# ygjwd12345/UCD

Hardware: AMD Instinct MI355X
Metric: images/sec (whole node) per UCD train step, VOC 15-5 step-1, 513^2 bs=24 (higher is better)
Workload: dtype bf16

## Files before the change

include/ucd_hip.h:

```cpp
#ifndef UCD_HIP_H
#define UCD_HIP_H

#include <stddef.h>
#include <stdint.h>

#ifdef __cplusplus
extern "C" {
#endif

#define UCD_VERSION 100

typedef void* ucd_stream_t;
typedef void* ucd_comm_t;

enum ucd_dtype { UCD_F32 = 0, UCD_BF16 = 1 };
enum ucd_act { UCD_ACT_IDENTITY = 0, UCD_ACT_LEAKY_RELU = 1, UCD_ACT_ELU = 2  };
#define UCD_ACT_MASK 0xff
#define UCD_NORM_ABS_GAMMA 0x100
enum ucd_pixcon_precision { UCD_PIXCON_F32 = 0, UCD_PIXCON_F16 = 1, UCD_PIXCON_F16_SPLIT = 2 };
enum ucd_error {
  UCD_OK = 0,
  UCD_EINVAL = -1,
  UCD_EALIGN = -2,
  UCD_EWORKSPACE = -3,
// ... 276 lines not shown

int ucd_conv3_tap_plan(int B, int H, int W, int dilation, int tile_rows, int* perm, int* masks, int* n_classes);
int ucd_conv3_tap_classes(int mode);
int ucd_conv3_tap_plans_resident(void);
int ucd_conv3_tap_stats(long long* launches, int* last_tile_rows, int* last_class_ordered);

int ucd_conv1x1_stats_finalize(const float* partial, int M, int C, const float* weight, float* running_mean,
                               float* running_var, float momentum, float eps, float* buf, float* pack, int flags,
                               ucd_stream_t stream);

int ucd_abn_reduce_partials(const float* partial, int tiles, int C, float* sums, float* sums_copy, const float* weight,
                            int flags, ucd_stream_t stream);

size_t ucd_conv1x1_wgrad_workspace_bytes(int M, int N, int K);
int ucd_conv1x1_wgrad(const void* dy, int ld_dy, const void* a, int lda, int M, int N, int K,
                      const float* in_mean, const float* in_scale, const float* in_shift, int in_act, float in_slope,
                      void* dw, void* workspace, size_t workspace_bytes, ucd_stream_t stream);

int ucd_abn_sync_finalize(const float* gathered, int world, int M, int C, const float* weight, float* running_mean,
                          float* running_var, float momentum, float eps, float* buf, int flags, ucd_stream_t stream);

int ucd_stem_conv7x7(const float* x, long long sb, long long sc, long long sh, long long sw, int B, int H, int W, const void* w,
                     void* z, ucd_stream_t stream);

int ucd_stem_conv_pool(const float* x, long long sb, long long sc, long long sh, long long sw, int B, int H, int W, const void* w,
                       const float* mean, const float* scale, const float* beta, int act, float slope, void* out, ucd_stream_t stream);
int ucd_stem_pooled_size(int n);
size_t ucd_stem_pool_workspace_bytes(int C);
int ucd_stem_apply_pool(const void* z, int B, int H, int W, int C, const float* mean, const float* scale, const float* beta, int act,
                        float slope, void* out, uint8_t* idx, ucd_stream_t stream);
int ucd_stem_pool_backward(const void* z, const void* dpool, const uint8_t* idx, int B, int H, int W, int C, const float* mean,
                           const float* invstd, const float* scale, const float* beta, const float* weight, float* sums, float count,
                           int act, float slope, void* dz, void* workspace, size_t workspace_bytes, int phase, ucd_stream_t stream);

size_t ucd_conv_wgrad_workspace_bytes(int M, int N, int K, int taps);
int ucd_conv_wgrad(const void* dz, int ld_dz, const void* x, int ld_x, int M, int N, int K, int taps, int H, int W, int dilation,
                   void* dw, float* dw32, int accumulate32, void* workspace, size_t workspace_bytes, ucd_stream_t stream);
int ucd_conv_wgrad_strided(const void* dz, int ld_dz, const void* x, int ld_x, int M, int N, int K, int taps, int H, int W,
                           int dilation, int stride, void* dw, float* dw32, int accumulate32, void* workspace, size_t workspace_bytes,
                           ucd_stream_t stream);
int ucd_conv_wgrad_ex(const void* dz, int ld_dz, const void* x, int ld_x, int M, int N, int K, int taps, int H, int W, int dilation,
                      int stride, void* dw, float* dw32, int accumulate32, void* workspace, size_t workspace_bytes, int flags,
                      ucd_stream_t stream);
int ucd_conv_wgrad_defer(int mode);
int ucd_conv_wgrad_mode(void);
int ucd_conv_wgrad_flush(ucd_stream_t stream);
int ucd_conv_wgrad_drop(ucd_stream_t stream);
int ucd_conv_wgrad_drop_all(void);

int ucd_flip_weights_batched(const void* src_flat, void* dst_flat, const int* blocks, int n_blocks, const long long* entries,
                             ucd_stream_t stream);
int ucd_flip_weights_batched64(const void* src_flat, void* dst_flat, const int* blocks, int n_blocks, const long long* entries,
                               ucd_stream_t stream);

int ucd_transpose_bf16(const void* src, int rows, int cols, void* dst, ucd_stream_t stream);

int ucd_conv_f32(const float* a, int lda, const float* w, int ldw, float* y, int ldy, int M, int N, int K, int taps, int H, int W,
                 int dilation, int accumulate, ucd_stream_t stream);
size_t ucd_conv_f32_wgrad_workspace_bytes(int M, int N, int K, int taps);
int ucd_conv_f32_wgrad(const float* dz, int ld_dz, const float* x, int ld_x, int M, int N, int K, int taps, int H, int W,
                       int dilation, float* dw, void* workspace, size_t workspace_bytes, ucd_stream_t stream);

#define UCD_SGD_MAX_GROUPS 8
typedef struct ucd_sgd_tensor {
  float* p;  const float* g;  float* m;  void* w16;
  long long n;
// ... 38 lines not shown
```

ucd_amd/abn.py:

```python
from __future__ import annotations

import os

from . import switches as _switches

import torch
import torch.distributed as dist
import torch.nn as nn
from torch.optim.optimizer import register_optimizer_step_post_hook

from . import hip
from .comm import direct_comm


def _act_code(name):
    try:
        return hip.ACT_CODES[name]
    except KeyError:
        raise RuntimeError(f"activation {name!r} is not supported by the HIP ABN (leaky_relu, elu, identity)") from None


_param_epoch = [0]


# ... 243 lines not shown
            sl = slice(o, o + c)
            dx = hip.empty_like_rows(x)
            hip.abn_bwd_apply(x, ld, dy[:, sl], ld_dy, None, 0, dx, c, None, 0, M, c, None, HW, mean[sl], invstd[sl],
                              scale[sl], shift[sl], weight[sl] if weight is not None else None,
                              sums[2 * o:2 * (o + c)], count, 0 if training else 1, act, slope)
            dxs.append(dx)
        return (dweight, dbias) + (None,) * 8 + tuple(dxs)


class _PlaneMean(torch.autograd.Function):

    @staticmethod
    def forward(ctx, x):
        x, M, Cc, HW, ld = hip.rows_view(x)
        B = x.shape[0]
        out = torch.empty(B, Cc, dtype=torch.float32, device=x.device)
        hip.plane_sum(x, ld, B, HW, Cc, 1.0 / HW, out)
        ctx.shape, ctx.dtype = x.shape, x.dtype
        return out.to(x.dtype).view(B, Cc, 1, 1)

    @staticmethod
    def backward(ctx, g):
        B, Cc, H, W = ctx.shape
        return (g.to(ctx.dtype) / (H * W)).expand(B, Cc, H, W)


def global_avg_pool(x):
    return _PlaneMean.apply(x)


class _StemABNPoolFunction(torch.autograd.Function):

    @staticmethod
    def forward(ctx, z, weight, bias, running_mean, running_var, training, momentum, eps, act, slope, group, eval_consts):
        B, Cc, H, W = z.shape
        M, HW = B * H * W, H * W
        zr, _, _, _, ld = hip.rows_view(z)
        dev = z.device
        world = _group_size(group) if training else 1
        sync = training and group is not False and (world > 1 or (_FORCE_SYNC and dist.is_initialized()))
        if training:
            buf = torch.empty(((8 + 2 * world) if sync else 6) * Cc, dtype=torch.float32, device=dev)
            if sync:
                pack = buf[6 * Cc:8 * Cc]
                hip.abn_sync_stats(zr, ld, M, Cc, None, HW, buf[:2 * Cc], buf[2 * Cc:3 * Cc], pack)
                comm = direct_comm(group)
                if comm is not None:
                    gathered = buf[8 * Cc:]
                    hip._check(hip.load().ucd_comm_all_gather(comm.handle, hip.ptr(pack), hip.ptr(gathered), 2 * Cc, hip.stream()),
                               "ucd_comm_all_gather")
                else:
                    gathered = _all_gather_stats(pack, world, group)
                hip.abn_sync_finalize(gathered, world, M, Cc, weight, running_mean, running_var, momentum, eps, buf, act)
            else:
                hip.abn_stats_finalize(zr, ld, M, Cc, None, HW, buf[:2 * Cc], buf[2 * Cc:3 * Cc], weight, running_mean, running_var,
                                       momentum, eps, buf[3 * Cc:4 * Cc], buf[4 * Cc:5 * Cc], buf[5 * Cc:6 * Cc], act)
            mean, invstd, scale = buf[3 * Cc:4 * Cc], buf[4 * Cc:5 * Cc], buf[5 * Cc:6 * Cc]
        else:
            mean, invstd, scale = running_mean, eval_consts[0], eval_consts[1]
        need_bwd = any(ctx.needs_input_grad[:3])
        out, idx = hip.stem_apply_pool(z, mean, scale, bias, act, slope, need_bwd)
        if need_bwd:
            ctx.save_for_backward(z, idx, weight, bias, mean, invstd, scale)
            ctx.cfg = (training, act, slope, group, world, sync, float(M * world))
        return out

    @staticmethod
    def backward(ctx, dp):
        z, idx, weight, bias, mean, invstd, scale = ctx.saved_tensors
        training, act, slope, group, world, sync, count = ctx.cfg
        if not training:
            raise RuntimeError("ucd_amd.abn: the fused stem has no frozen-statistics backward (fix_bn keeps the separate layers)")
        Cc = z.shape[1]
        if dp.dtype != z.dtype:
            dp = dp.to(z.dtype)
        if not dp.is_contiguous(memory_format=torch.channels_last):
            dp = dp.contiguous(memory_format=torch.channels_last)
        sums = torch.empty(2 * Cc, dtype=torch.float32, device=z.device)
        dz = torch.empty_like(z) if ctx.needs_input_grad[0] else None
        if not sync:
            hip.stem_pool_backward(z, dp, idx, mean, invstd, scale, bias, weight, sums, count, act, slope, dz, 3 if dz is not None else 1)
            dbias, dweight = sums[:Cc], sums[Cc:]
        else:
            hip.stem_pool_backward(z, dp, idx, mean, invstd, scale, bias, weight, sums, count, act, slope, None, 1)
            local = sums.clone()
            dbias, dweight = local[:Cc], local[Cc:]
            comm = direct_comm(group)
            if comm is not None:
                hip._check(hip.load().ucd_comm_all_reduce_sum(comm.handle, hip.ptr(sums), 2 * Cc, hip.stream()), "ucd_comm_all_reduce_sum")
            else:
                _all_reduce_sums(sums, group)
            if dz is not None:
                hip.stem_pool_backward(z, dp, idx, mean, invstd, scale, bias, weight, sums, count, act, slope, dz, 2)
        return (dz, dweight if weight is not None else None, dbias if bias is not None else None) + (None,) * 9


def stem_norm_pool(bn, z):
    import os
    if _switches.get("UCD_STEM_FOLD", "1") == "0" or not getattr(bn, "ucd_fused_abn", False):
        return None
    Cc = z.shape[1] if z.dim() == 4 else 0
    if not (z.is_cuda and z.dim() == 4 and z.dtype == torch.bfloat16 and z.is_contiguous(memory_format=torch.channels_last)
            and z.shape[2] > 2 and z.shape[3] > 2 and Cc % 8 == 0 and 2048 % max(Cc, 1) == 0
            and bn.activation in ("leaky_relu", "identity")):
        return None
    needs_grad = torch.is_grad_enabled() and (z.requires_grad or (bn.weight is not None and bn.weight.requires_grad))
    if needs_grad and not bn.training:
        return None
    act = _act_code(bn.activation) | (hip.NORM_ABS_GAMMA if bn._abs_gamma else 0)
    if bn.training:
        bn.__dict__.pop("_eval_cache", None)
    return _StemABNPoolFunction.apply(z, bn.weight, bn.bias, bn.running_mean, bn.running_var, bn.training, bn.momentum, bn.eps, act,
                                      bn.activation_param, bn._group(), None if bn.training else bn._eval_constants())


class ABN(nn.Module):

    ucd_fused_abn = True
    _inplace_contract = False
    _sync = False
    _abs_gamma = False

    def __init__(self, num_features, eps=1e-5, momentum=0.1, affine=True, activation="leaky_relu",
                 activation_param=0.01, group=None):
        super().__init__()
        self.num_features, self.eps, self.momentum, self.affine = num_features, eps, momentum, affine
        self.activation, self.activation_param = activation, activation_param
        self.group = group
        if affine:
            self.weight = nn.Parameter(torch.ones(num_features))
            self.bias = nn.Parameter(torch.zeros(num_features))
        else:
            self.register_parameter("weight", None)
            self.register_parameter("bias", None)
        self.register_buffer("running_mean", torch.zeros(num_features))
        self.register_buffer("running_var", torch.ones(num_features))

    def reset_parameters(self):
        nn.init.constant_(self.running_mean, 0)
        nn.init.constant_(self.running_var, 1)
        if self.affine:
            nn.init.constant_(self.weight, 1)
            nn.init.constant_(self.bias, 0)

    def _group(self):
        return self.group if self._sync else False
# ... 82 lines not shown
```

ucd_amd/backbone.py:

```python
from __future__ import annotations

import sys
from collections import OrderedDict
from functools import partial

import torch
import torch.nn as nn

from . import switches as _switches
from .blocks import Conv2d, ResidualBlock, try_index

_STAGE_DILATION = {16: (1, 1, 1, 2), 8: (1, 1, 2, 4)}


class GlobalAvgPool2d(nn.Module):

    def forward(self, inputs):
        return inputs.flatten(2).mean(dim=2)


class ResNet(nn.Module):
    def __init__(self, structure, bottleneck, norm_act=nn.BatchNorm2d, classes=0,
                 output_stride=16, keep_outputs=False):
        super().__init__()
# ... 19 lines not shown
                blocks[f"block{b + 1}"] = ResidualBlock(cin, width, norm_act=norm_act, stride=stride, dilation=d)
                cin = width[-1]
            self.add_module(f"mod{stage + 2}", nn.Sequential(blocks))
            width = tuple(2 * c for c in width)
        self.out_channels = cin

        if classes != 0:
            self.classifier = nn.Sequential(OrderedDict(
                [("avg_pool", GlobalAvgPool2d()), ("fc", nn.Linear(cin, classes))]))

    def _stem(self, x):
        m = self.mod1
        if hasattr(m, "pool1") and getattr(m.bn1, "ucd_fused_abn", False) and x.is_cuda:
            pool = m.pool1
            if (pool.kernel_size, pool.stride, pool.padding, pool.dilation, pool.ceil_mode) == (3, 2, 1, 1, False):
                from .abn import stem_norm_pool
                y = _stem_eval_fused(m.conv1, m.bn1, x)
                if y is not None:
                    return y
                z = _stem_conv(m.conv1, x)
                y = stem_norm_pool(m.bn1, z)
                return y if y is not None else pool(m.bn1(z))
        return m(x)

    def forward(self, x):
        outs = [self._stem(x)]
        for name in ("mod2", "mod3", "mod4", "mod5"):
            outs.append(getattr(self, name)(outs[-1]))
        if hasattr(self, "classifier"):
            outs.append(self.classifier(outs[-1]))
        return outs if self.keep_outputs else outs[-1]


class _StemConvFunction(torch.autograd.Function):

    @staticmethod
    def forward(ctx, x, w):
        from . import hip
        ctx.save_for_backward(x, w)
        return hip.stem_conv7x7(x, w)

    @staticmethod
    def backward(ctx, dz):
        x, w = ctx.saved_tensors
        dw = None
        if ctx.needs_input_grad[1]:
            xb = x.to(torch.bfloat16).contiguous(memory_format=torch.channels_last)
            dw = torch.ops.aten.convolution_backward(dz.contiguous(memory_format=torch.channels_last), xb, w, None, [2, 2], [3, 3],
                                                     [1, 1], False, [0, 0], 1, [False, True, False])[1]
        return None, dw


def _stem_conv(conv, x):
    w = conv.working_weight() if hasattr(conv, "working_weight") else None
    if w is None and x.is_cuda and torch.is_autocast_enabled() and torch.get_autocast_dtype("cuda") == torch.bfloat16:
        w = conv.weight.to(torch.bfloat16)
    if (w is None or not x.is_cuda or x.dim() != 4 or x.dtype != torch.float32 or x.requires_grad or conv.bias is not None
            or tuple(conv.weight.shape) != (64, 3, 7, 7) or conv.stride != (2, 2) or conv.padding != (3, 3)
            or conv.dilation != (1, 1) or w.dtype != torch.bfloat16 or not w.is_contiguous(memory_format=torch.channels_last)
            or _switches.get("UCD_OWN_STEM", "1") == "0"):
        return conv(x)
    if torch.is_grad_enabled() and w.requires_grad:
        return _StemConvFunction.apply(x, w)
    from . import hip
    return hip.stem_conv7x7(x, w)


def _stem_eval_fused(conv, bn, x):
    from . import abn as _abn
    if (torch.is_grad_enabled() or bn.training or _switches.get("UCD_STEM_EVAL_FUSED", "1") == "0" or _switches.get("UCD_OWN_STEM", "1") == "0"
            or _switches.get("UCD_STEM_FOLD", "1") == "0" or not getattr(bn, "ucd_fused_abn", False)
            or bn.activation not in ("leaky_relu", "identity")):
        return None
    w = conv.working_weight() if hasattr(conv, "working_weight") else None
    if w is None and x.is_cuda and torch.is_autocast_enabled() and torch.get_autocast_dtype("cuda") == torch.bfloat16:
        w = conv.weight.to(torch.bfloat16)
    if (w is None or not x.is_cuda or x.dim() != 4 or x.dtype != torch.float32 or conv.bias is not None
            or tuple(conv.weight.shape) != (64, 3, 7, 7) or conv.stride != (2, 2) or conv.padding != (3, 3) or conv.dilation != (1, 1)
            or w.dtype != torch.bfloat16 or not w.is_contiguous(memory_format=torch.channels_last) or x.shape[2] < 8 or x.shape[3] < 8):
        return None
    from . import hip
    invstd, scale = bn._eval_constants()
    return hip.stem_conv_pool(x, w, bn.running_mean, scale, bn.bias, _abn._act_code(bn.activation), bn.activation_param)


_NETS = {
    "18": ([2, 2, 2, 2], False), "34": ([3, 4, 6, 3], False), "50": ([3, 4, 6, 3], True),
    "101": ([3, 4, 23, 3], True), "152": ([3, 8, 36, 3], True),
}
__all__ = ["ResNet"]
for _n, (_s, _b) in _NETS.items():
    setattr(sys.modules[__name__], f"net_resnet{_n}", partial(ResNet, structure=_s, bottleneck=_b))
    __all__.append(f"net_resnet{_n}")
```

ucd_amd/csrc/stem.hip:

```cpp
#include "common.h"

namespace ucd {
namespace {

typedef __hip_bfloat16 bf16;
constexpr int kThreads = 256;
constexpr int kRedBlocks = 1024;
constexpr int kApplyRows = 4;

__device__ __forceinline__ float leaky(float z, float slope) { return z > 0.f ? z : z * slope; }
__device__ __forceinline__ float bf16_round(float v) { return __bfloat162float(__float2bfloat16(v)); }

struct StemArgs {
  const bf16* z; int B, H, W, C, PH, PW;
  const float *mean, *scale, *beta, *invstd, *weight, *sums;
  float slope, inv_count;
  int abs_gamma, cg_shift;
};

__global__ __launch_bounds__(kThreads) void stem_apply_pool_kernel(StemArgs p, bf16* __restrict__ out, uint8_t* __restrict__ idx) {
  const int cgs = p.cg_shift, CG = 1 << cgs;
  const int t = blockIdx.x * kThreads + threadIdx.x;
  const int cg = t & (CG - 1), pw = t >> cgs, ph = blockIdx.y, b = blockIdx.z;
  if (pw >= p.PW) return;
  const size_t pix = ((size_t)b * p.PH + ph) * p.PW + pw;
  float mu[8], sc[8], sh[8], best[8];
  int bi[8];
#pragma unroll
  for (int e = 0; e < 8; ++e) {
    mu[e] = p.mean[cg * 8 + e]; sc[e] = p.scale[cg * 8 + e]; sh[e] = p.beta ? p.beta[cg * 8 + e] : 0.f;
    best[e] = -INFINITY; bi[e] = 0;
  }
  Vec<bf16> v[9];
// ... 401 lines not shown
          union { bf16 v[4]; uint2 u; } o;
#pragma unroll
          for (int e = 0; e < 4; ++e) {
            const float zq = bf16_round(acc[a][c][g * 4 + e]);
            o.v[e] = __float2bfloat16(leaky((zq - m4[e]) * s4[e] + b4[e], q.slope));
          }
          if (!inside) o.u = make_uint2(0xFF80FF80u, 0xFF80FF80u);
          *reinterpret_cast<uint2*>(dst + ch) = o.u;
        }
    }
    __syncthreads();
    for (int i = tid; i < kFPH * kFPW * 8; i += kThreads) {
      const int cg = i & 7, pp = i >> 3, pr = pp / kFPW, pc = pp - pr * kFPW;
      const int ph = (oy0 + 1) / 2 + pr, pw = (ox0 + 1) / 2 + pc;
      if (ph >= q.PH || pw >= q.PW) continue;
      float best[8];
#pragma unroll
      for (int e = 0; e < 8; ++e) best[e] = -INFINITY;
#pragma unroll
      for (int kh = 0; kh < 3; ++kh)
#pragma unroll
        for (int kw = 0; kw < 3; ++kw) {
          Vec<bf16> v;
          v.raw = *reinterpret_cast<const uint4*>(Tl + ((2 * pr + kh) * kSTW + 2 * pc + kw) * kFTP + cg * 8);
#pragma unroll
          for (int e = 0; e < 8; ++e) best[e] = fmaxf(best[e], v.get(e));
        }
      Vec<bf16> o;
#pragma unroll
      for (int e = 0; e < 8; ++e) o.set(e, best[e]);
      o.store(q.out + (((size_t)b * q.PH + ph) * q.PW + pw) * 64 + cg * 8);
    }
  }
}

bool stem_args_ok(const void* z, int B, int H, int W, int C) {
  return z && B > 0 && B < 65536 && H > 1 && H < 65536 && W > 1 && C >= 8 && (C & (C - 1)) == 0 && C <= 2048 && aligned16(z);
}

}
}

using namespace ucd;

extern "C" {

int ucd_stem_pooled_size(int n) { return (n + 2 - 3) / 2 + 1; }

size_t ucd_stem_pool_workspace_bytes(int C) { return (size_t)kRedBlocks * 2 * C * sizeof(float); }

int ucd_stem_apply_pool(const void* z, int B, int H, int W, int C, const float* mean, const float* scale, const float* beta, int act,
                        float slope, void* out, uint8_t* idx, ucd_stream_t stream) {
  static const char* fn = "ucd_stem_apply_pool";
  UCD_REQUIRE(stem_args_ok(z, B, H, W, C) && mean && scale && out && aligned16(out) && (!idx || (reinterpret_cast<uintptr_t>(idx) & 7) == 0),
              UCD_EINVAL, "%s: dense channels-last bf16 maps with a power-of-two channel count in 8..2048 expected", fn);
  const int a = act & UCD_ACT_MASK;
  UCD_REQUIRE(a != UCD_ACT_ELU, UCD_EUNSUPPORTED, "%s: leaky_relu / identity only (an elu stem keeps the separate passes)", fn);
  StemArgs p{};
  p.z = (const bf16*)z; p.B = B; p.H = H; p.W = W; p.C = C; p.PH = ucd_stem_pooled_size(H); p.PW = ucd_stem_pooled_size(W);
  p.mean = mean; p.scale = scale; p.beta = beta; p.slope = a == UCD_ACT_IDENTITY ? 1.f : slope;
  p.cg_shift = __builtin_ctz(C / 8);
  stem_apply_pool_kernel<<<dim3(ceil_div(p.PW * (C / 8), kThreads), p.PH, B), kThreads, 0, (hipStream_t)stream>>>(p, (bf16*)out, idx);
  return check_launch(fn);
}

int ucd_stem_conv7x7(const float* x, long long sb, long long sc, long long sh, long long sw, int B, int H, int W, const void* w,
// ... 33 lines not shown

int ucd_stem_pool_backward(const void* z, const void* dpool, const uint8_t* idx, int B, int H, int W, int C, const float* mean,
                           const float* invstd, const float* scale, const float* beta, const float* weight, float* sums, float count,
                           int act, float slope, void* dz, void* workspace, size_t workspace_bytes, int phase, ucd_stream_t stream) {
  static const char* fn = "ucd_stem_pool_backward";
  UCD_REQUIRE(stem_args_ok(z, B, H, W, C) && dpool && idx && mean && invstd && scale && sums && aligned16(dpool), UCD_EINVAL,
              "%s: bad arguments", fn);
  UCD_REQUIRE(phase >= 1 && phase <= 3 && (!(phase & 2) || (dz && aligned16(dz) && count > 0.f)), UCD_EINVAL, "%s: bad phase / dz", fn);
  const int a = act & UCD_ACT_MASK;
  UCD_REQUIRE(a != UCD_ACT_ELU, UCD_EUNSUPPORTED, "%s: leaky_relu / identity only", fn);
  StemArgs p{};
  p.z = (const bf16*)z; p.B = B; p.H = H; p.W = W; p.C = C; p.PH = ucd_stem_pooled_size(H); p.PW = ucd_stem_pooled_size(W);
  p.mean = mean; p.scale = scale; p.beta = beta; p.invstd = invstd; p.weight = weight; p.sums = sums;
  p.slope = a == UCD_ACT_IDENTITY ? 1.f : slope; p.abs_gamma = (act & UCD_NORM_ABS_GAMMA) != 0;
  p.cg_shift = __builtin_ctz(C / 8);
  hipStream_t s = (hipStream_t)stream;
  if (phase & 1) {
    UCD_REQUIRE(workspace && workspace_bytes >= ucd_stem_pool_workspace_bytes(C), UCD_EWORKSPACE, "%s: workspace too small", fn);
    stem_pool_bwd_reduce_kernel<<<kRedBlocks, kThreads, kThreads * 16 * sizeof(float), s>>>(p, (const bf16*)dpool, idx, (float*)workspace);
    int rc = check_launch(fn);
    if (rc) return rc;
    stem_sum_partials_kernel<<<2 * C, kThreads, 0, s>>>((const float*)workspace, kRedBlocks, C, p.abs_gamma ? weight : nullptr, sums);
    rc = check_launch(fn);
    if (rc) return rc;
  }
  if (phase & 2) {
    p.inv_count = 1.f / count;
    stem_pool_bwd_apply_kernel<<<dim3(ceil_div(((W + 1) / 2) * (C / 8), kThreads), ceil_div(H, kApplyRows), B), kThreads, 0, s>>>(p, (const bf16*)dpool, idx, (bf16*)dz);
    return check_launch(fn);
  }
  return 0;
}

}
```

ucd_amd/hip.py:

```python
from __future__ import annotations

import ctypes as C
import os

import torch

_HERE = os.path.dirname(os.path.abspath(__file__))
LIB_PATH = os.path.join(_HERE, "libucd_hip.so")

F32, BF16 = 0, 1
ACT_IDENTITY, ACT_LEAKY_RELU, ACT_ELU = 0, 1, 2
ACT_CODES = {"identity": ACT_IDENTITY, "leaky_relu": ACT_LEAKY_RELU, "elu": ACT_ELU}
ACT_MASK = 0xFF
NORM_ABS_GAMMA = 0x100
PIX_TILE = 128
PIXCON_LD = 256
PIXCON_F32, PIXCON_F16, PIXCON_F16_SPLIT = 0, 1, 2
KD_UNBIASED, KD_PLAIN = 0, 1
EUNSUPPORTED = -4
SEG_FORMS = {1: "pk<16,8>", 2: "pk<20,4>", 3: "pk<12,12>", 4: "reg<24,16>", 5: "reg<24,24>", 6: "wide/fixed", 7: "wide/f32"}
PIXCON_PATHS = {1: "f32", 2: "f32/wide", 3: "f16/planned", 4: "f16/split"}
PIXCON_PRECISION = {"f32": PIXCON_F32, "fp32": PIXCON_F32, "f16": PIXCON_F16, "fp16": PIXCON_F16,
                    "f16_split": PIXCON_F16_SPLIT}

# ... 63 lines not shown
    "ucd_abn_sync_backward_comm": (_i, [_p, _i, _p, _i, _p, _i, _p, _i, _p, _i, _p, _i, _i, _i, _i, _p, _i, _p, _p, _p, _p, _p,
                                        _p, _p, _i, _f, _p, _z, _p]),
    "ucd_abn_sync_stats": (_i, [_p, _i, _i, _i, _i, _p, _i, _p, _p, _p, _p, _z, _p]),
    "ucd_abn_sync_forward": (_i, [_p, _i, _p, _i, _p, _i, _i, _i, _i, _p, _i, _p, _i, _p, _p, _p, _p, _f, _f, _p, _i, _f, _p]),
    "ucd_abn_sync_bwd_reduce": (_i, [_p, _i, _p, _i, _p, _i, _i, _i, _i, _p, _i, _p, _p, _p, _p, _p, _i, _f, _p, _p, _p, _z, _p]),
    "ucd_abn_bwd_apply": (_i, [_p, _i, _p, _i, _p, _i, _p, _i, _p, _i, _i, _i, _i, _p, _i, _p, _p, _p, _p, _p, _p,
                               _f, _i, _i, _f, _p]),
    "ucd_abn_forward": (_i, [_p, _i, _p, _i, _p, _i, _i, _i, _i, _p, _i, _p, _p, _p, _p, _f, _f, _i, _p, _p, _i, _f, _p, _z, _p]),
    "ucd_abn_backward": (_i, [_p, _i, _p, _i, _p, _i, _p, _i, _p, _i, _i, _i, _i, _p, _i, _p, _p, _p, _p, _p, _p, _f, _i, _i,
                              _i, _f, _p, _z, _p]),
    "ucd_plane_sum": (_i, [_p, _i, _i, _i, _i, _i, _f, _p, _p]),
    "ucd_window_mean_workspace_bytes": (_z, [_i, _i, _i, _i, _i]),
    "ucd_window_mean": (_i, [_p, _i, _i, _i, _i, _i, _i, _i, _i, _p, _i, _p, _z, _p]),
    "ucd_attmap_workspace_bytes": (_z, [_i, _i]),
    "ucd_attmap": (_i, [_p, _i, _p, _i, _i, _i, _i, _i, _p, _z, _p]),
    "ucd_attn_mse_workspace_bytes": (_z, [_i, _i]),
    "ucd_attn_mse": (_i, [_p, _i, _p, _i, _i, _i, _i, _i, _f, _p, _p, _i, _p, _z, _p]),
    "ucd_conv1x1_row_tiles": (_i, [_i]),
    "ucd_conv1x1_stats_partial_bytes": (_z, [_i, _i]),
    "ucd_conv1x1": (_i, [C.POINTER(Conv1x1Desc), _p]),
    "ucd_conv1x1_stats_finalize": (_i, [_p, _i, _i, _p, _p, _p, _f, _f, _p, _p, _i, _p]),
    "ucd_conv3_tap_plan": (_i, [_i, _i, _i, _i, _i, _p, _p, _p]),
    "ucd_conv3_tap_classes": (_i, [_i]),
    "ucd_conv3_tap_plans_resident": (_i, []),
    "ucd_conv3_tap_stats": (_i, [_p, _p, _p]),
    "ucd_abn_reduce_partials": (_i, [_p, _i, _i, _p, _p, _p, _i, _p]),
    "ucd_conv1x1_wgrad_workspace_bytes": (_z, [_i, _i, _i]),
    "ucd_conv1x1_wgrad": (_i, [_p, _i, _p, _i, _i, _i, _i, _p, _p, _p, _i, _f, _p, _p, _z, _p]),
    "ucd_abn_sync_finalize": (_i, [_p, _i, _i, _i, _p, _p, _p, _f, _f, _p, _i, _p]),
    "ucd_stem_pooled_size": (_i, [_i]),
    "ucd_stem_pool_workspace_bytes": (_z, [_i]),
    "ucd_stem_apply_pool": (_i, [_p, _i, _i, _i, _i, _p, _p, _p, _i, _f, _p, _p, _p]),
    "ucd_stem_pool_backward": (_i, [_p, _p, _p, _i, _i, _i, _i, _p, _p, _p, _p, _p, _p, _f, _i, _f, _p, _p, _z, _i, _p]),
    "ucd_conv_wgrad_workspace_bytes": (_z, [_i, _i, _i, _i]),
    "ucd_conv_wgrad": (_i, [_p, _i, _p, _i, _i, _i, _i, _i, _i, _i, _i, _p, _p, _i, _p, _z, _p]),
    "ucd_stem_conv7x7": (_i, [_p, C.c_longlong, C.c_longlong, C.c_longlong, C.c_longlong, _i, _i, _i, _p, _p, _p]),
    "ucd_stem_conv_pool": (_i, [_p, C.c_longlong, C.c_longlong, C.c_longlong, C.c_longlong, _i, _i, _i, _p, _p, _p, _p, _i, _f, _p, _p]),
    "ucd_conv_wgrad_strided": (_i, [_p, _i, _p, _i, _i, _i, _i, _i, _i, _i, _i, _i, _p, _p, _i, _p, _z, _p]),
    "ucd_conv_wgrad_ex": (_i, [_p, _i, _p, _i, _i, _i, _i, _i, _i, _i, _i, _i, _p, _p, _i, _p, _z, _i, _p]),
    "ucd_conv_wgrad_defer": (_i, [_i]),
    "ucd_conv_wgrad_mode": (_i, []),
    "ucd_conv_wgrad_flush": (_i, [_p]),
    "ucd_conv_wgrad_drop": (_i, [_p]),
    "ucd_conv_wgrad_drop_all": (_i, []),
    "ucd_transpose_bf16": (_i, [_p, _i, _i, _p, _p]),
    "ucd_conv_f32": (_i, [_p, _i, _p, _i, _p, _i, _i, _i, _i, _i, _i, _i, _i, _i, _p]),
    "ucd_conv_f32_wgrad_workspace_bytes": (_z, [_i, _i, _i, _i]),
    "ucd_conv_f32_wgrad": (_i, [_p, _i, _p, _i, _i, _i, _i, _i, _i, _i, _i, _p, _p, _z, _p]),
    "ucd_flip_weights_batched": (_i, [_p, _p, _p, _i, _p, _p]),
    "ucd_flip_weights_batched64": (_i, [_p, _p, _p, _i, _p, _p]),
    "ucd_sgd_chunk": (_i, []),
    "ucd_sgd_step": (_i, [_p, _p, _i, _p, _p]),
    "ucd_sgd_hyper_store": (_i, [_p, _p, _p]),
    "ucd_sgd_step_dev": (_i, [_p, _p, _i, _p, _p]),
    "ucd_reg_chunk": (_i, []),
    "ucd_reg_hyper_store": (_i, [_p, _p, _p]),
    "ucd_reg_step": (_i, [_p, _p, _i, _i, _p, _p, _p, _p]),
    "ucd_pixcon_prep_workspace_bytes": (_z, [_i, _i]),
    "ucd_pixcon_prep": (_i, [_p, _i, _i, _i, _i, _i, _i, _p, _i, _i, _i, _i, _p, _p, _p, _p, _p, _p, _z, _p]),
    "ucd_pixcon_gather": (_i, [_p, _i, _p, _i, _i, _i, _i, _p, _p, _p, _i, _p, _p, _i, _p, _i, _p, _p, _p, _p]),
    "ucd_pixcon_loss_workspace_bytes": (_z, [_i, _i, _i]),
    "ucd_pixcon_loss_plan": (_i, [_i, _i, _i, _i, _f, _p, _p, _p, _p, _p, _p, _p]),
    "ucd_pixcon_loss": (_i, [_p, _i, _i, _p, _p, _i, _i, _p, _p, _i, _p, _i, _f, _i, _i, _p, _p, _i, _p, _p, _z, _p]),
    "ucd_pixcon_loss_given_p": (_i, [_p, _i, _i, _p, _p, _i, _p, _i, _f, _i, _p, _p, _i, _p, _p, _z, _p]),
    "ucd_pixcon_scatter_grad": (_i, [_p, _p, _i, _p, _p, _p, _p, _p, _i, _i, _i, _i, _p]),
    "ucd_seg_confusion": (_i, [_p, _i, _p, _i, _i, _i, _i, _i, _i, _i, _p, _p, _p]),
# ... 505 lines not shown
    PH, PW = lib.ucd_stem_pooled_size(OH), lib.ucd_stem_pooled_size(OW)
    out = torch.empty((B, 64, PH, PW), dtype=torch.bfloat16, device=x.device, memory_format=torch.channels_last)
    sb, sc, sh, sw = x.stride()
    with _timed("ucd_stem_conv7x7", x.numel() * 4 + out.numel() * 2):
        _check(lib.ucd_stem_conv_pool(ptr(x), sb, sc, sh, sw, B, H, W, ptr(w), ptr(mean), ptr(scale), ptr(beta), act, float(slope),
                                      ptr(out), stream()), "ucd_stem_conv_pool")
    return out


def stem_apply_pool(z, mean, scale, beta, act, slope, want_idx):
    lib = load()
    B, Cc, H, W = z.shape
    PH, PW = lib.ucd_stem_pooled_size(H), lib.ucd_stem_pooled_size(W)
    out = torch.empty((B, Cc, PH, PW), dtype=z.dtype, device=z.device, memory_format=torch.channels_last)
    idx = torch.empty((B, PH, PW, Cc), dtype=torch.uint8, device=z.device) if want_idx else None
    with _timed("ucd_stem_apply_pool", (z.numel() + out.numel()) * 2 + (idx.numel() if idx is not None else 0)):
        _check(lib.ucd_stem_apply_pool(ptr(z), B, H, W, Cc, ptr(mean), ptr(scale), ptr(beta), act, float(slope), ptr(out), ptr(idx),
                                       stream()), "ucd_stem_apply_pool")
    return out, idx


def stem_pool_backward(z, dpool, idx, mean, invstd, scale, beta, weight, sums, count, act, slope, dz, phase):
    lib = load()
    B, Cc, H, W = z.shape
    nbytes = lib.ucd_stem_pool_workspace_bytes(Cc)
    ws = workspace(nbytes, z.device)
    work = (z.numel() * (2 if phase & 1 else 0) + (2 * z.numel() * 2 if phase & 2 else 0) + dpool.numel() * 3 * (1 + (phase == 3)))
    with _timed("ucd_stem_pool_backward", work):
        _check(lib.ucd_stem_pool_backward(ptr(z), ptr(dpool), ptr(idx), B, H, W, Cc, ptr(mean), ptr(invstd), ptr(scale), ptr(beta),
                                          ptr(weight), ptr(sums), float(count), act, float(slope), ptr(dz), ptr(ws), nbytes,
                                          int(phase), stream()), "ucd_stem_pool_backward")


def wgrad_defer(mode):
    return int(load().ucd_conv_wgrad_defer(int(mode) & 3))


def _wgrad_side_release(stream=None):
    from . import abn as _abn
    node = _abn._abn_node()
    if node is not None:
        node.wgrad_side_release(stream)


def wgrad_flush():
    s = stream()
    _check(load().ucd_conv_wgrad_flush(s), "ucd_conv_wgrad_flush")
    _wgrad_side_release(s)


def wgrad_drop():
    s = stream()
    rc = load().ucd_conv_wgrad_drop(s)
    if rc == 0:
        _wgrad_side_release(s)
    return rc


def wgrad_drop_all():
    rc = load().ucd_conv_wgrad_drop_all()
    if rc == 0:
        _wgrad_side_release()
    return rc


_wgrad_turn = {}
# ... 86 lines not shown
```

ucd_amd/switches.py:

```python
from __future__ import annotations

import os

DEFAULTS = {
    "UCD_FUSED_CONV1X1": "1",
    "UCD_BWD_LINK": "1",
    "UCD_BLOCK_LINK": "1",
    "UCD_PROJ_ALIAS": "1",
    "UCD_DGRAD_VIA_FWD": "1",
    "UCD_LIB_GEMM_WIDE": "0",
    "UCD_OWN3X3_MIN_TILES": "1",
    "UCD_OWN3X3_WIDE": "1",
    "UCD_OWN_STRIDED": "1",
    "UCD_OWN_WGRAD": "1",
    "UCD_F32_OWN_CONV": "0",
    "UCD_OWN_HEADS": "1",
    "UCD_OWN_STEM": "1",
    "UCD_WGRAD3": "1",
    "UCD_CONV_PIPE": "auto",
    "UCD_CONV_BN64_TILES": "128",
    "UCD_CONV_LW64_TILES": "128",
    "UCD_WGRAD_DEFER": "1",
    "UCD_WGRAD_STREAM": "1",
    "UCD_CONV3_TAP_CLASSES": "1",
    "UCD_CONV3_MIN_ROWS": "0",
    "UCD_STAT_ATOMIC": "1",
    "UCD_SEG_PK": "1",
    "UCD_SEG_KD_EX": "1",
    "UCD_FUSED_LDE": "1",
    "UCD_STEM_EVAL_FUSED": "1",
    "UCD_STEM_FOLD": "1",
    "UCD_ABN_NODE": "1",
    "UCD_SGD": "hip",
    "UCD_STEP_GRAPH": "auto",
    "UCD_TEACHER_OVERLAP": "1",
    "UCD_DIRECT_RCCL": "1",
    "UCD_IPC_SYNC": "auto",
    "UCD_IPC_TIMEOUT_MS": "60000",
    "UCD_DDP_LATE_COPY": "1",
    "UCD_DDP_DIRECT": "auto",
    "UCD_FORCE_COLLECTIVES": "0",
}

_cache: dict = {}


def get(name: str, default: str | None = None) -> str:
    v = _cache.get(name)
    if v is None:
        if default is None:
            default = DEFAULTS.get(name, "")
        v = _cache[name] = os.environ.get(name, default)
    return v


def set(name: str, value) -> None:
    os.environ[name] = str(value)
    _cache[name] = str(value)


def unset(name: str) -> None:
    os.environ.pop(name, None)
    _cache.pop(name, None)

# ... 8 lines not shown
```

Baseline: 846.2.

## Fuse stem norm-pool backward with conv1 weight gradient in one MFMA kernel

Adds a HIP kernel that computes the stem ABN+maxpool backward dz tile in LDS and immediately contracts it with the input image patch into per-workgroup 7x7 weight-gradient slabs, followed by a reduction kernel. The dz tensor is never written to memory, and the separate aten convolution_backward for conv1's weight is replaced by a placeholder handoff between the two autograd functions. This avoids the full-resolution dz write and read plus a library wgrad call. In exchange it adds fp32 slab workspace, a reduction pass and coupling logic that errors out if conv1's output has another consumer.

```diff
diff --git a/include/ucd_hip.h b/include/ucd_hip.h
--- a/include/ucd_hip.h
+++ b/include/ucd_hip.h
@@ -332,6 +332,13 @@
 int ucd_stem_pool_backward(const void* z, const void* dpool, const uint8_t* idx, int B, int H, int W, int C, const float* mean,
                            const float* invstd, const float* scale, const float* beta, const float* weight, float* sums, float count,
                            int act, float slope, void* dz, void* workspace, size_t workspace_bytes, int phase, ucd_stream_t stream);
+
+size_t ucd_stem_wgrad_workspace_bytes(int max_workgroups);
+int ucd_stem_pool_backward_wgrad(const void* z, const void* dpool, const uint8_t* idx, int B, int H, int W, int C, const float* mean,
+                                 const float* invstd, const float* scale, const float* beta, const float* weight, const float* sums,
+                                 float count, int act, float slope, const float* x, long long sb, long long sc, long long sh,
+                                 long long sw, int IH, int IW, void* dw, void* workspace, size_t workspace_bytes, void* dz,
+                                 int max_workgroups, ucd_stream_t stream);
 
 size_t ucd_conv_wgrad_workspace_bytes(int M, int N, int K, int taps);
 int ucd_conv_wgrad(const void* dz, int ld_dz, const void* x, int ld_x, int M, int N, int K, int taps, int H, int W, int dilation,
diff --git a/ucd_amd/abn.py b/ucd_amd/abn.py
--- a/ucd_amd/abn.py
+++ b/ucd_amd/abn.py
@@ -299,7 +299,7 @@
 class _StemABNPoolFunction(torch.autograd.Function):
 
     @staticmethod
-    def forward(ctx, z, weight, bias, running_mean, running_var, training, momentum, eps, act, slope, group, eval_consts):
+    def forward(ctx, z, weight, bias, running_mean, running_var, training, momentum, eps, act, slope, group, eval_consts, link=None):
         B, Cc, H, W = z.shape
         M, HW = B * H * W, H * W
         zr, _, _, _, ld = hip.rows_view(z)
@@ -330,6 +330,7 @@
         if need_bwd:
             ctx.save_for_backward(z, idx, weight, bias, mean, invstd, scale)
             ctx.cfg = (training, act, slope, group, world, sync, float(M * world))
+            ctx.stem_link = link
         return out
 
     @staticmethod
@@ -344,7 +345,10 @@
         if not dp.is_contiguous(memory_format=torch.channels_last):
             dp = dp.contiguous(memory_format=torch.channels_last)
         sums = torch.empty(2 * Cc, dtype=torch.float32, device=z.device)
-        dz = torch.empty_like(z) if ctx.needs_input_grad[0] else None
+        link = ctx.stem_link
+        fuse = (link is not None and ctx.needs_input_grad[0] and Cc == 64 and link.w.requires_grad and not z.retains_grad
+                and not z._backward_hooks and _switches.get("UCD_STEM_WGRAD", "1") != "0")
+        dz = torch.empty_like(z) if (ctx.needs_input_grad[0] and not fuse) else None
         if not sync:
             hip.stem_pool_backward(z, dp, idx, mean, invstd, scale, bias, weight, sums, count, act, slope, dz, 3 if dz is not None else 1)
             dbias, dweight = sums[:Cc], sums[Cc:]
@@ -359,7 +363,10 @@
                 _all_reduce_sums(sums, group)
             if dz is not None:
                 hip.stem_pool_backward(z, dp, idx, mean, invstd, scale, bias, weight, sums, count, act, slope, dz, 2)
-        return (dz, dweight if weight is not None else None, dbias if bias is not None else None) + (None,) * 9
+        if fuse:
+            link.dw = hip.stem_pool_backward_wgrad(z, dp, idx, mean, invstd, scale, bias, weight, sums, count, act, slope, link.x, link.w)
+            dz = link.placeholder
+        return (dz, dweight if weight is not None else None, dbias if bias is not None else None) + (None,) * 10
 
 
 def stem_norm_pool(bn, z):
@@ -378,7 +385,8 @@
     if bn.training:
         bn.__dict__.pop("_eval_cache", None)
     return _StemABNPoolFunction.apply(z, bn.weight, bn.bias, bn.running_mean, bn.running_var, bn.training, bn.momentum, bn.eps, act,
-                                      bn.activation_param, bn._group(), None if bn.training else bn._eval_constants())
+                                      bn.activation_param, bn._group(), None if bn.training else bn._eval_constants(),
+                                      getattr(z, "_ucd_stem_link", None))
 
 
 class ABN(nn.Module):
diff --git a/ucd_amd/backbone.py b/ucd_amd/backbone.py
--- a/ucd_amd/backbone.py
+++ b/ucd_amd/backbone.py
@@ -75,23 +75,60 @@
         return outs if self.keep_outputs else outs[-1]
 
 
+class _StemLink:
+    __slots__ = ("x", "w", "dw", "placeholder")
+
+    def __init__(self, x, w):
+        self.x, self.w, self.dw, self.placeholder = x, w, None, None
+
+    def offer(self, z):
+        self.placeholder = _zero_scalar(z).expand(z.shape)
+        z._ucd_stem_link = self
+
+    def is_placeholder(self, g):
+        ph = self.placeholder
+        return g is ph or (ph is not None and g.data_ptr() == ph.data_ptr() and g.shape == ph.shape and not any(g.stride()))
+
+
+_zeros = {}
+
+
+def _zero_scalar(z):
+    if torch.cuda.is_current_stream_capturing():
+        return torch.zeros((), dtype=z.dtype, device=z.device)
+    key = (z.device, z.dtype)
+    t = _zeros.get(key)
+    if t is None:
+        t = _zeros[key] = torch.zeros((), dtype=z.dtype, device=z.device)
+    return t
+
+
 class _StemConvFunction(torch.autograd.Function):
 
     @staticmethod
-    def forward(ctx, x, w):
+    def forward(ctx, x, w, link):
         from . import hip
         ctx.save_for_backward(x, w)
+        ctx.link = link
         return hip.stem_conv7x7(x, w)
 
     @staticmethod
     def backward(ctx, dz):
         x, w = ctx.saved_tensors
+        link = ctx.link
+        if link is not None and link.dw is not None:
+            dw, link.dw = link.dw, None
+            if not link.is_placeholder(dz):
+                raise RuntimeError("ucd stem: the norm + pool backward took over conv1's weight gradient, but the gradient that arrived "
+                                   "at conv1 is not its placeholder - the convolution's output has a second consumer.  Run with "
+                                   "UCD_STEM_WGRAD=0")
+            return None, dw, None
         dw = None
         if ctx.needs_input_grad[1]:
             xb = x.to(torch.bfloat16).contiguous(memory_format=torch.channels_last)
             dw = torch.ops.aten.convolution_backward(dz.contiguous(memory_format=torch.channels_last), xb, w, None, [2, 2], [3, 3],
                                                      [1, 1], False, [0, 0], 1, [False, True, False])[1]
-        return None, dw
+        return None, dw, None
 
 
 def _stem_conv(conv, x):
@@ -104,7 +141,11 @@
             or _switches.get("UCD_OWN_STEM", "1") == "0"):
         return conv(x)
     if torch.is_grad_enabled() and w.requires_grad:
-        return _StemConvFunction.apply(x, w)
+        link = _StemLink(x, w) if _switches.get("UCD_STEM_WGRAD", "1") != "0" else None
+        z = _StemConvFunction.apply(x, w, link)
+        if link is not None:
+            link.offer(z)
+        return z
     from . import hip
     return hip.stem_conv7x7(x, w)
 
diff --git a/ucd_amd/csrc/stem.hip b/ucd_amd/csrc/stem.hip
--- a/ucd_amd/csrc/stem.hip
+++ b/ucd_amd/csrc/stem.hip
@@ -1,4 +1,5 @@
 #include "common.h"
+#include "stem_plan.h"
 
 namespace ucd {
 namespace {
@@ -466,6 +467,236 @@
       o.store(q.out + (((size_t)b * q.PH + ph) * q.PW + pw) * 64 + cg * 8);
     }
   }
+}
+
+constexpr int kWTP = 72;
+constexpr int kWSeg = 36;
+static_assert(6 * kWSeg == kSIP, "a patch row holds 2 parities x 3 channels");
+
+struct StemWgradArgs {
+  StemArgs a;
+  const bf16* dpool; const uint8_t* idx;
+  const float* x; long long sb, sc, sh, sw; int IH, IW;
+  bf16* dz;
+  float* slab;
+  int tiles_y, tiles_x, ntiles;
+};
+
+__global__ __launch_bounds__(kThreads, 2) void stem_pool_bwd_wgrad_kernel(StemWgradArgs q) {
+  typedef float f32x16 __attribute__((ext_vector_type(16)));
+  typedef __bf16 bf16x8 __attribute__((ext_vector_type(8)));
+  typedef __bf16 bf16x4 __attribute__((ext_vector_type(4)));
+  typedef __attribute__((address_space(3))) bf16x4* lds_bf16x4;
+  const StemArgs& p = q.a;
+  __shared__ __attribute__((aligned(16))) unsigned short Tl[kSTH * kSTW * kWTP];
+  __shared__ __attribute__((aligned(16))) unsigned short In[kSIR * kSIP];
+  __shared__ __attribute__((aligned(16))) float Pl[3 * 64];
+  const int tid = threadIdx.x, lane = tid & 63, wave = __builtin_amdgcn_readfirstlane(tid >> 6);
+
+  const int cg = tid & 7, il = (tid >> 3) & 15, rg = tid >> 7;
+  if (tid < 64) {
+    const int ch = tid;
+    const float scv = p.scale[ch], isv = p.invstd[ch];
+    float k1v = p.sums[p.C + ch] * p.inv_count, gwv;
+    if (p.abs_gamma) {
+      if (p.weight && p.weight[ch] < 0.f) k1v = -k1v;
+      gwv = scv;
+    } else {
+      gwv = (p.weight ? p.weight[ch] : 1.f) * isv;
+    }
+    Pl[ch] = p.sums[ch] * p.inv_count; Pl[64 + ch] = k1v; Pl[128 + ch] = gwv;
+  }
+  float mu[8], sc[8], sh[8], is[8];
+#pragma unroll
+  for (int e = 0; e < 8; ++e) {
+    const int ch = cg * 8 + e;
+    mu[e] = p.mean[ch]; sc[e] = p.scale[ch]; sh[e] = p.beta ? p.beta[ch] : 0.f; is[e] = p.invstd[ch];
+  }
+
+  const int fe = tid < kSIP ? tid : kSIP - 1, fpx = fe / 3, fc = fe - fpx * 3;
+  const int fdst = (fpx & 1) * 3 * kWSeg + fc * kWSeg + (fpx >> 1);
+  float pre[kSIR];
+  unsigned premask = 0;
+  auto origin = [&](int tile, int& b, int& oy0, int& ox0) {
+    b = tile / (q.tiles_y * q.tiles_x);
+    const int rem = tile - b * q.tiles_y * q.tiles_x;
+    oy0 = (rem / q.tiles_x) * kSTH;
+    ox0 = (rem % q.tiles_x) * kSTW;
+  };
+  auto fetch = [&](int tile) {
+    unsigned okm = 0;
+    int b, oy0, ox0;
+    origin(tile, b, oy0, ox0);
+    const int ix = 2 * ox0 - 3 + fpx;
+    const bool colok = fpx < 2 * kSTW + 5 && (unsigned)ix < (unsigned)q.IW;
+    const float* src = q.x + b * q.sb + fc * q.sc + (colok ? ix : 0) * q.sw;
+#pragma unroll
+    for (int r = 0; r < kSIR; ++r) {
+      const int iy = 2 * oy0 - 3 + r;
+      const bool ok = colok && (unsigned)iy < (unsigned)q.IH;
+      pre[r] = src[(ok ? iy : 0) * q.sh];
+      okm |= ok ? (1u << r) : 0u;
+    }
+    premask = okm;
+  };
+
+  const int r32 = lane & 31, h = lane >> 5, nb = wave & 1, tb0 = (wave >> 1) * 3, ntb = (wave >> 1) ? 2 : 3;
+  int boff[3];
+  unsigned bsh[3];
+#pragma unroll
+  for (int tb = 0; tb < 3; ++tb) {
+    int t = (tb0 + tb) * 32 + r32;
+    t = t < 147 ? t : 146;
+    const int ky = t / 21, j = t - ky * 21, kx = j / 3, c = j - kx * 3;
+    const int e = ky * kSIP + (kx & 1) * 3 * kWSeg + c * kWSeg + (kx >> 1) + 8 * h;
+    boff[tb] = e >> 1;
+    bsh[tb] = (e & 1) * 16;
+  }
+  const int aoff = (8 * h + ((lane & 15) >> 2)) * kWTP + nb * 32 + 16 * ((lane >> 4) & 1) + 4 * (lane & 3);
+  f32x16 acc[3];
+#pragma unroll
+  for (int tb = 0; tb < 3; ++tb)
+#pragma unroll
+    for (int i = 0; i < 16; ++i) acc[tb][i] = 0.f;
+
+  if ((int)blockIdx.x < q.ntiles) fetch(blockIdx.x);
+  for (int tile = blockIdx.x; tile < q.ntiles; tile += gridDim.x) {
+    int b, oy0, ox0;
+    origin(tile, b, oy0, ox0);
+    __syncthreads();
+    if (tid < kSIP) {
+#pragma unroll
+      for (int r = 0; r < kSIR; ++r) {
+        const bf16 v = __float2bfloat16((premask >> r) & 1u ? pre[r] : 0.f);
+        In[r * kSIP + fdst] = *reinterpret_cast<const unsigned short*>(&v);
+      }
+    }
+    {
+      const int i = (ox0 >> 1) + il, phb = (oy0 >> 1) + 2 * rg, y0 = oy0 + kApplyRows * rg, x0 = 2 * i;
+      Vec<bf16> g[3][2], v[kApplyRows][2];
+      uint2 w[3][2];
+      bool gv[3][2];
+#pragma unroll
+      for (int a = 0; a < 3; ++a)
+#pragma unroll
+        for (int c = 0; c < 2; ++c) {
+          gv[a][c] = phb + a < p.PH && i + c < p.PW;
+          const size_t off = (((size_t)b * p.PH + min(phb + a, p.PH - 1)) * p.PW + min(i + c, p.PW - 1)) * p.C + cg * 8;
+          w[a][c] = *reinterpret_cast<const uint2*>(q.idx + off);
+          g[a][c].load(q.dpool + off);
+        }
+#pragma unroll
+      for (int r = 0; r < kApplyRows; ++r) {
+        if (!(r & 1)) {
+#pragma unroll
+          for (int rr = r; rr < r + 2; ++rr)
+#pragma unroll
+            for (int cx = 0; cx < 2; ++cx)
+              v[rr][cx].load(p.z + (((size_t)b * p.H + min(y0 + rr, p.H - 1)) * p.W + min(x0 + cx, p.W - 1)) * p.C + cg * 8);
+        }
+#pragma unroll
+        for (int cx = 0; cx < 2; ++cx) {
+          const bool inside = y0 + r < p.H && x0 + cx < p.W;
+          float dy[8] = {0.f, 0.f, 0.f, 0.f, 0.f, 0.f, 0.f, 0.f};
+#pragma unroll
+          for (int ya = 0; ya < 2; ++ya) {
+            if (ya == 1 && !(r & 1)) continue;
+            const int a = (r >> 1) + ya, kh = (r & 1) ? (ya ? 0 : 2) : 1;
+#pragma unroll
+            for (int xa = 0; xa < 2; ++xa) {
+              if (xa == 1 && !cx) continue;
+              const int kw = cx ? (xa ? 0 : 2) : 1;
+              const unsigned pos = gv[a][xa] ? (unsigned)(kh * 3 + kw) : 0xffu;
+#pragma unroll
+              for (int e = 0; e < 8; ++e) {
+                const unsigned id = ((e < 4 ? w[a][xa].x : w[a][xa].y) >> (8 * (e & 3))) & 0xffu;
+                dy[e] += id == pos ? g[a][xa].get(e) : 0.f;
+              }
+            }
+          }
+          Vec<bf16> o;
+          int ko = cg * 8;
+          asm volatile("" : "+v"(ko));
+          const float *k0 = Pl + ko, *k1 = k0 + 64, *gw = k0 + 128;
+#pragma unroll
+          for (int e = 0; e < 8; ++e) {
+            const float xc = v[r][cx].get(e) - mu[e];
+            const float dza = dy[e] * (xc * sc[e] + sh[e] > 0.f ? 1.f : p.slope);
+            o.set(e, (dza - k0[e] - (xc * is[e]) * k1[e]) * gw[e]);
+          }
+          if (!inside) o.raw = make_uint4(0u, 0u, 0u, 0u);
+          *reinterpret_cast<uint4*>(&Tl[((kApplyRows * rg + r) * kSTW + 2 * il + cx) * kWTP + cg * 8]) = o.raw;
+          if (q.dz && inside) o.store(q.dz + (((size_t)b * p.H + y0 + r) * p.W + x0 + cx) * p.C + cg * 8);
+          __builtin_amdgcn_sched_barrier(0);
+        }
+      }
+    }
+    __syncthreads();
+    if (tile + (int)gridDim.x < q.ntiles) fetch(tile + gridDim.x);
+#pragma unroll
+    for (int ks = 0; ks < 16; ++ks) {
+      const unsigned short* ap = &Tl[ks * 16 * kWTP + aoff];
+      const bf16x4 lo = __builtin_amdgcn_ds_read_tr16_b64_v4bf16((lds_bf16x4)ap);
+      const bf16x4 hi = __builtin_amdgcn_ds_read_tr16_b64_v4bf16((lds_bf16x4)(ap + 4 * kWTP));
+      bf16x8 af;
+      af[0] = lo[0]; af[1] = lo[1]; af[2] = lo[2]; af[3] = lo[3];
+      af[4] = hi[0]; af[5] = hi[1]; af[6] = hi[2]; af[7] = hi[3];
+      const unsigned* rowp = reinterpret_cast<const unsigned*>(In) + (2 * (ks >> 1) * kSIP + 16 * (ks & 1)) / 2;
+#pragma unroll
+      for (int tb = 0; tb < 3; ++tb) {
+        if (tb < ntb) {
+          const unsigned* s = rowp + boff[tb];
+          const unsigned d0 = s[0], d1 = s[1], d2 = s[2], d3 = s[3], d4 = s[4];
+          union { unsigned u[4]; bf16x8 v; } f;
+          f.u[0] = __builtin_amdgcn_alignbit(d1, d0, bsh[tb]);
+          f.u[1] = __builtin_amdgcn_alignbit(d2, d1, bsh[tb]);
+          f.u[2] = __builtin_amdgcn_alignbit(d3, d2, bsh[tb]);
+          f.u[3] = __builtin_amdgcn_alignbit(d4, d3, bsh[tb]);
+          acc[tb] = __builtin_amdgcn_mfma_f32_32x32x16_bf16(af, f.v, acc[tb], 0, 0, 0);
+        }
+      }
+    }
+  }
+  float* dst = q.slab + (size_t)blockIdx.x * kStemWgradOut;
+#pragma unroll
+  for (int tb = 0; tb < 3; ++tb) {
+    const int t = (tb0 + tb) * 32 + r32;
+    if (tb >= ntb || t >= 147) continue;
+#pragma unroll
+    for (int i = 0; i < 16; ++i) dst[(nb * 32 + (i & 3) + 8 * (i >> 2) + 4 * h) * 147 + t] = acc[tb][i];
+  }
+}
+
+__global__ __launch_bounds__(kThreads) void stem_wgrad_sum_kernel(const float* __restrict__ slab, int nslabs, bf16* __restrict__ dw) {
+  __shared__ float4 red[kThreads];
+  const int col = threadIdx.x & 7, sl = threadIdx.x >> 3;
+  const float4* src = reinterpret_cast<const float4*>(slab) + blockIdx.x * 8 + col;
+  float4 s = make_float4(0.f, 0.f, 0.f, 0.f);
+#pragma unroll 8
+  for (int g = sl; g < nslabs; g += 32) {
+    const float4 v = src[(size_t)g * (kStemWgradOut / 4)];
+    s.x += v.x; s.y += v.y; s.z += v.z; s.w += v.w;
+  }
+  red[threadIdx.x] = s;
+  __syncthreads();
+  if (sl == 0) {
+    for (int l = 1; l < 32; ++l) {
+      const float4 v = red[l * 8 + col];
+      s.x += v.x; s.y += v.y; s.z += v.z; s.w += v.w;
+    }
+    bf16* dst = dw + (blockIdx.x * 8 + col) * 4;
+    dst[0] = __float2bfloat16(s.x); dst[1] = __float2bfloat16(s.y); dst[2] = __float2bfloat16(s.z); dst[3] = __float2bfloat16(s.w);
+  }
+}
+static_assert(kStemWgradOut % 32 == 0, "the slab sum walks 32 outputs per workgroup");
+
+int device_cus() {
+  int dev = 0, n = 0;
+  if (hipGetDevice(&dev) != hipSuccess || hipDeviceGetAttribute(&n, hipDeviceAttributeMultiprocessorCount, dev) != hipSuccess) {
+    (void)hipGetLastError();
+    return 0;
+  }
+  return n;
 }
 
 bool stem_args_ok(const void* z, int B, int H, int W, int C) {
@@ -565,4 +796,38 @@
   return 0;
 }
 
-}
+size_t ucd_stem_wgrad_workspace_bytes(int max_workgroups) { return stem_wgrad_workspace_bound(device_cus(), max_workgroups); }
+
+int ucd_stem_pool_backward_wgrad(const void* z, const void* dpool, const uint8_t* idx, int B, int H, int W, int C, const float* mean,
+                                 const float* invstd, const float* scale, const float* beta, const float* weight, const float* sums,
+                                 float count, int act, float slope, const float* x, long long sb, long long sc, long long sh,
+                                 long long sw, int IH, int IW, void* dw, void* workspace, size_t workspace_bytes, void* dz,
+                                 int max_workgroups, ucd_stream_t stream) {
+  static const char* fn = "ucd_stem_pool_backward_wgrad";
+  UCD_REQUIRE(stem_args_ok(z, B, H, W, C) && C == 64 && dpool && idx && mean && invstd && scale && sums && aligned16(dpool) &&
+              (reinterpret_cast<uintptr_t>(idx) & 7) == 0 && count > 0.f && (!dz || aligned16(dz)), UCD_EINVAL, "%s: bad arguments", fn);
+  UCD_REQUIRE(x && dw && (reinterpret_cast<uintptr_t>(dw) & 1) == 0 && IH > 0 && IW > 0 && H == (IH - 1) / 2 + 1 && W == (IW - 1) / 2 + 1 &&
+              max_workgroups >= 0, UCD_EINVAL, "%s: the image [B, 3, %d, %d] does not give a %d x %d map", fn, IH, IW, H, W);
+  const int a = act & UCD_ACT_MASK;
+  UCD_REQUIRE(a != UCD_ACT_ELU, UCD_EUNSUPPORTED, "%s: leaky_relu / identity only", fn);
+  const StemWgradPlan plan = stem_wgrad_plan(B, H, W, device_cus(), max_workgroups);
+  UCD_REQUIRE(plan.grid > 0, UCD_EINVAL, "%s: no plan for this map / device", fn);
+  UCD_REQUIRE(workspace && aligned16(workspace) && workspace_bytes >= plan.workspace_bytes, UCD_EWORKSPACE, "%s: workspace too small", fn);
+  StemWgradArgs q{};
+  StemArgs& p = q.a;
+  p.z = (const bf16*)z; p.B = B; p.H = H; p.W = W; p.C = C; p.PH = ucd_stem_pooled_size(H); p.PW = ucd_stem_pooled_size(W);
+  p.mean = mean; p.scale = scale; p.beta = beta; p.invstd = invstd; p.weight = weight; p.sums = sums;
+  p.slope = a == UCD_ACT_IDENTITY ? 1.f : slope; p.abs_gamma = (act & UCD_NORM_ABS_GAMMA) != 0;
+  p.cg_shift = __builtin_ctz(C / 8);
+  p.inv_count = 1.f / count;
+  q.dpool = (const bf16*)dpool; q.idx = idx; q.x = x; q.sb = sb; q.sc = sc; q.sh = sh; q.sw = sw; q.IH = IH; q.IW = IW;
+  q.dz = (bf16*)dz; q.slab = (float*)workspace; q.tiles_y = plan.tiles_y; q.tiles_x = plan.tiles_x; q.ntiles = plan.ntiles;
+  hipStream_t s = (hipStream_t)stream;
+  stem_pool_bwd_wgrad_kernel<<<plan.grid, kThreads, 0, s>>>(q);
+  int rc = check_launch(fn);
+  if (rc) return rc;
+  stem_wgrad_sum_kernel<<<kStemWgradOut / 32, kThreads, 0, s>>>((const float*)workspace, plan.grid, (bf16*)dw);
+  return check_launch(fn);
+}
+
+}
diff --git a/ucd_amd/csrc/stem_plan.h b/ucd_amd/csrc/stem_plan.h
--- /dev/null
+++ b/ucd_amd/csrc/stem_plan.h
@@ -0,0 +1,41 @@
+#pragma once
+#include <stddef.h>
+
+namespace ucd {
+
+constexpr int kStemTileH = 8, kStemTileW = 32;
+constexpr int kStemWgradOut = 64 * 147;
+constexpr int kStemWgradPerCU = 2;
+constexpr int kStemWgradMaxGrid = 2048;
+
+struct StemWgradPlan {
+  int tiles_y, tiles_x, ntiles, grid;
+  size_t workspace_bytes;
+};
+
+inline StemWgradPlan stem_wgrad_plan(int B, int OH, int OW, int cus, int max_workgroups) {
+  StemWgradPlan p{0, 0, 0, 0, 0};
+  if (B <= 0 || OH <= 0 || OW <= 0 || cus <= 0 || max_workgroups < 0) return p;
+  p.tiles_y = (OH + kStemTileH - 1) / kStemTileH;
+  p.tiles_x = (OW + kStemTileW - 1) / kStemTileW;
+  const long long n = (long long)B * p.tiles_y * p.tiles_x;
+  if (n > 0x7fffffffLL) return p;
+  p.ntiles = (int)n;
+  long long g = (long long)cus * kStemWgradPerCU;
+  if (g > kStemWgradMaxGrid) g = kStemWgradMaxGrid;
+  if (max_workgroups > 0 && max_workgroups < g) g = max_workgroups;
+  if (g > n) g = n;
+  p.grid = (int)g;
+  p.workspace_bytes = (size_t)p.grid * kStemWgradOut * sizeof(float);
+  return p;
+}
+
+inline size_t stem_wgrad_workspace_bound(int cus, int max_workgroups) {
+  if (cus <= 0 || max_workgroups < 0) return 0;
+  long long g = (long long)cus * kStemWgradPerCU;
+  if (g > kStemWgradMaxGrid) g = kStemWgradMaxGrid;
+  if (max_workgroups > 0 && max_workgroups < g) g = max_workgroups;
+  return (size_t)g * kStemWgradOut * sizeof(float);
+}
+
+}
diff --git a/ucd_amd/hip.py b/ucd_amd/hip.py
--- a/ucd_amd/hip.py
+++ b/ucd_amd/hip.py
@@ -119,6 +119,9 @@
     "ucd_stem_pool_workspace_bytes": (_z, [_i]),
     "ucd_stem_apply_pool": (_i, [_p, _i, _i, _i, _i, _p, _p, _p, _i, _f, _p, _p, _p]),
     "ucd_stem_pool_backward": (_i, [_p, _p, _p, _i, _i, _i, _i, _p, _p, _p, _p, _p, _p, _f, _i, _f, _p, _p, _z, _i, _p]),
+    "ucd_stem_wgrad_workspace_bytes": (_z, [_i]),
+    "ucd_stem_pool_backward_wgrad": (_i, [_p, _p, _p, _i, _i, _i, _i, _p, _p, _p, _p, _p, _p, _f, _i, _f, _p, C.c_longlong, C.c_longlong,
+                                          C.c_longlong, C.c_longlong, _i, _i, _p, _p, _z, _p, _i, _p]),
     "ucd_conv_wgrad_workspace_bytes": (_z, [_i, _i, _i, _i]),
     "ucd_conv_wgrad": (_i, [_p, _i, _p, _i, _i, _i, _i, _i, _i, _i, _i, _p, _p, _i, _p, _z, _p]),
     "ucd_stem_conv7x7": (_i, [_p, C.c_longlong, C.c_longlong, C.c_longlong, C.c_longlong, _i, _i, _i, _p, _p, _p]),
@@ -690,6 +693,23 @@
                                           int(phase), stream()), "ucd_stem_pool_backward")
 
 
+def stem_pool_backward_wgrad(z, dpool, idx, mean, invstd, scale, beta, weight, sums, count, act, slope, x, w, dz=None, max_workgroups=0):
+    lib = load()
+    B, Cc, H, W = z.shape
+    _, _, IH, IW = x.shape
+    dw = torch.empty_like(w)
+    nbytes = lib.ucd_stem_wgrad_workspace_bytes(int(max_workgroups))
+    ws = workspace(nbytes, z.device, "stem_wgrad")
+    sb, sc, sh, sw = x.stride()
+    work = z.numel() * 2 * (1 + (dz is not None)) + dpool.numel() * 3 + x.numel() * 4
+    with _timed("ucd_stem_pool_backward_wgrad", work):
+        _check(lib.ucd_stem_pool_backward_wgrad(ptr(z), ptr(dpool), ptr(idx), B, H, W, Cc, ptr(mean), ptr(invstd), ptr(scale), ptr(beta),
+                                                ptr(weight), ptr(sums), float(count), act, float(slope), ptr(x), sb, sc, sh, sw, IH, IW,
+                                                ptr(dw), ptr(ws), nbytes, ptr(dz), int(max_workgroups), stream()),
+               "ucd_stem_pool_backward_wgrad")
+    return dw
+
+
 def wgrad_defer(mode):
     return int(load().ucd_conv_wgrad_defer(int(mode) & 3))
 
diff --git a/ucd_amd/switches.py b/ucd_amd/switches.py
--- a/ucd_amd/switches.py
+++ b/ucd_amd/switches.py
@@ -30,6 +30,7 @@
     "UCD_FUSED_LDE": "1",
     "UCD_STEM_EVAL_FUSED": "1",
     "UCD_STEM_FOLD": "1",
+    "UCD_STEM_WGRAD": "1",
     "UCD_ABN_NODE": "1",
     "UCD_SGD": "hip",
     "UCD_STEP_GRAPH": "auto",
```

After: 851.0, median of 6. Within noise of the previous version (+0.6%).
